# zhm1205/Multimodal_TTA

Hardware: AMD Instinct MI355X
Metric: adapted volumes/sec (higher is better)
Workload: dtype bf16

## Files before the change

include/mmtta.h:

```cpp
#ifndef MMTTA_H
#define MMTTA_H

#include <stdint.h>

#ifdef __cplusplus
extern "C" {
#endif

#define MMTTA_ABI_VERSION 2

typedef enum {
  MMTTA_OK = 0,
  MMTTA_ERR_INVALID = -1,
  MMTTA_ERR_UNSUPPORTED = -2,
  MMTTA_ERR_LAUNCH = -3,
  MMTTA_ERR_WORKSPACE = -4
} mmtta_status;

typedef enum { MMTTA_F32 = 0, MMTTA_BF16 = 1 } mmtta_dtype;

typedef struct {
  void* ptr;
  int32_t n, c, d, h, w;
  int64_t sn, sc, sd, sh, sw;
// ... 18 lines not shown
  float negative_slope;
  int32_t _pad2;
} mmtta_norm_on_load;

const char* mmtta_last_error(void);
int mmtta_abi_version(void);

#define MMTTA_OPT_PROFILE_MAIN_KERNEL_ONLY 1
#define MMTTA_OPT_SPLITK_BELOW 2
#define MMTTA_OPT_SPLITK_TARGET 3
#define MMTTA_OPT_WGRAD_WORKGROUPS 4
#define MMTTA_OPT_WGRAD_THIN_SLABS 5
#define MMTTA_OPT_IGEMM_PIPELINE 6
#define MMTTA_OPT_EPILOGUE_VEC16 9
#define MMTTA_OPT_IGEMM_LEAN 10
#define MMTTA_OPT_WGRAD_VECTOR_STAGING 11
#define MMTTA_OPT_CLASS_FUSED_MIN_WORKGROUPS 12
#define MMTTA_OPT_THIN_MFMA 13
#define MMTTA_OPT_IGEMM_FRAGMENT_REUSE 14
#define MMTTA_OPT_LAME_TILED 15
#define MMTTA_OPT_RAW_STAGING 16
#define MMTTA_OPT_HEAD_LOSS_PAIR 17
#define MMTTA_OPT_THIN_LEAN 18
int mmtta_set_option(int key, int value);

int mmtta_copy_strided(const mmtta_tensor* src, const mmtta_tensor* dst, void* stream);

typedef enum {
  MMTTA_CONV_FWD = 0,
  MMTTA_CONV_DGRAD = 1,
  MMTTA_CONVT_FWD = 2,
  MMTTA_CONVT_DGRAD = 3
} mmtta_conv_op;

typedef struct {
  int32_t op;
  int32_t ksize;
  int32_t stride;
  int32_t cin;
  int32_t cout;
  int32_t dtype;
} mmtta_conv_desc;

int64_t mmtta_conv_packed_bytes(const mmtta_conv_desc* desc);

int mmtta_conv_pack_weights(const mmtta_conv_desc* desc, const float* w_master, void* packed, void* stream);
// ... 18 lines not shown
} mmtta_conv_plan_t;

int mmtta_conv_plan(const mmtta_conv_desc* desc, const mmtta_tensor* x, const mmtta_tensor* y,
                    mmtta_conv_plan_t* plan);

typedef struct {
  const mmtta_tensor* add;
  mmtta_norm_on_load add_norm;
} mmtta_conv_epilogue;

int mmtta_conv_run(const mmtta_conv_desc* desc, const mmtta_tensor* x, const mmtta_norm_on_load* x_norm,
                   const void* packed, const float* bias, const mmtta_conv_epilogue* epi,
                   const mmtta_tensor* y, int accumulate, float* stats, void* workspace,
                   int64_t workspace_bytes, void* stream);

int mmtta_conv_route(const mmtta_conv_desc* desc, const mmtta_tensor* x, const mmtta_norm_on_load* x_norm,
                     const mmtta_conv_epilogue* epi, const mmtta_tensor* y, int accumulate, const float* stats);

int mmtta_conv_stages_raw(const mmtta_conv_desc* desc, const mmtta_tensor* x, const mmtta_norm_on_load* x_norm,
                          const mmtta_conv_epilogue* epi, const mmtta_tensor* y, int accumulate, const float* stats);

int mmtta_conv_thin_lean(const mmtta_conv_desc* desc, const mmtta_tensor* x, const mmtta_norm_on_load* x_norm,
                         const mmtta_conv_epilogue* epi, const mmtta_tensor* y, int accumulate, const float* stats);

typedef struct {
  int32_t items_per_set;
  int32_t inner;
  int64_t packed_outer, packed_inner;
  int64_t weight_outer, weight_inner;
  int64_t bias_outer, bias_inner;
} mmtta_param_sets;

int mmtta_conv_run_sets(const mmtta_conv_desc* desc, const mmtta_tensor* x, const mmtta_norm_on_load* x_norm,
                        const void* packed, const float* bias, const mmtta_conv_epilogue* epi,
                        const mmtta_tensor* y, int accumulate, float* stats, void* workspace,
                        int64_t workspace_bytes, const mmtta_param_sets* sets, void* stream);

int mmtta_conv_head_loss_eligible(const mmtta_conv_desc* desc, const mmtta_tensor* x, const mmtta_norm_on_load* x_norm,
                                  const mmtta_conv_epilogue* epi, const mmtta_tensor* y, const mmtta_tensor* dlogits,
                                  int softmax, int per_item);
int64_t mmtta_conv_head_loss_partials(const mmtta_conv_desc* desc, const mmtta_tensor* x, const mmtta_tensor* y);
int mmtta_conv_head_loss_run_sets(const mmtta_conv_desc* desc, const mmtta_tensor* x, const mmtta_norm_on_load* x_norm,
                                  const void* packed, const float* bias, const mmtta_conv_epilogue* epi,
                                  const mmtta_tensor* y, const mmtta_tensor* dlogits, int softmax, int per_item,
                                  double* partial, float* loss, const mmtta_param_sets* sets, void* stream);

// ... 294 lines not shown
```

multimodal_tta_amd/_lib.py:

```python
from __future__ import annotations

import ctypes as C
import os
from typing import Optional, Sequence

import torch

_HERE = os.path.dirname(os.path.abspath(__file__))
LIB_PATH = os.path.join(_HERE, "csrc", "libmmtta.so")

F32, BF16 = 0, 1
CONV_FWD, CONV_DGRAD, CONVT_FWD, CONVT_DGRAD = 0, 1, 2, 3
NORM_INSTANCE, NORM_BATCH, NORM_GROUP = 0, 1, 2


class MmttaError(RuntimeError):
    pass


class Tensor(C.Structure):
    _fields_ = [
        ("ptr", C.c_void_p),
        ("n", C.c_int32), ("c", C.c_int32), ("d", C.c_int32), ("h", C.c_int32), ("w", C.c_int32),
        ("sn", C.c_int64), ("sc", C.c_int64), ("sd", C.c_int64), ("sh", C.c_int64), ("sw", C.c_int64),
# ... 79 lines not shown


_P = C.POINTER
_SIGNATURES = {
    "mmtta_last_error": (C.c_char_p, []),
    "mmtta_abi_version": (C.c_int, []),
    "mmtta_set_option": (C.c_int, [C.c_int, C.c_int]),
    "mmtta_intensity_scratch_bytes": (C.c_int64, [C.c_int]),
    "mmtta_intensity_normalize": (C.c_int, [_P(Tensor), _P(IntensityRule), _P(Tensor), C.c_void_p, C.c_void_p]),
    "mmtta_copy_strided": (C.c_int, [_P(Tensor), _P(Tensor), C.c_void_p]),
    "mmtta_conv_packed_bytes": (C.c_int64, [_P(ConvDesc)]),
    "mmtta_conv_pack_weights": (C.c_int, [_P(ConvDesc), C.c_void_p, C.c_void_p, C.c_void_p]),
    "mmtta_conv_pack_table_bytes": (C.c_int64, [C.c_int]),
    "mmtta_conv_pack_table_build": (C.c_int, [_P(PackItem), C.c_int, C.c_void_p, _P(C.c_int64)]),
    "mmtta_conv_pack_batched": (C.c_int, [C.c_void_p, C.c_int, C.c_int64, C.c_void_p]),
    "mmtta_conv_plan": (C.c_int, [_P(ConvDesc), _P(Tensor), _P(Tensor), _P(ConvPlan)]),
    "mmtta_conv_run": (C.c_int, [_P(ConvDesc), _P(Tensor), _P(NormOnLoad), C.c_void_p, C.c_void_p, _P(ConvEpilogue),
                                 _P(Tensor), C.c_int, C.c_void_p, C.c_void_p, C.c_int64, C.c_void_p]),
    "mmtta_conv_run_sets": (C.c_int, [_P(ConvDesc), _P(Tensor), _P(NormOnLoad), C.c_void_p, C.c_void_p, _P(ConvEpilogue),
                                      _P(Tensor), C.c_int, C.c_void_p, C.c_void_p, C.c_int64, _P(ParamSets), C.c_void_p]),
    "mmtta_conv_route": (C.c_int, [_P(ConvDesc), _P(Tensor), _P(NormOnLoad), _P(ConvEpilogue), _P(Tensor), C.c_int, C.c_void_p]),
    "mmtta_conv_stages_raw": (C.c_int, [_P(ConvDesc), _P(Tensor), _P(NormOnLoad), _P(ConvEpilogue), _P(Tensor), C.c_int, C.c_void_p]),
    "mmtta_conv_thin_lean": (C.c_int, [_P(ConvDesc), _P(Tensor), _P(NormOnLoad), _P(ConvEpilogue), _P(Tensor), C.c_int, C.c_void_p]),
    "mmtta_conv_head_loss_eligible": (C.c_int, [_P(ConvDesc), _P(Tensor), _P(NormOnLoad), _P(ConvEpilogue), _P(Tensor), _P(Tensor),
                                                C.c_int, C.c_int]),
    "mmtta_conv_head_loss_partials": (C.c_int64, [_P(ConvDesc), _P(Tensor), _P(Tensor)]),
    "mmtta_conv_head_loss_run_sets": (C.c_int, [_P(ConvDesc), _P(Tensor), _P(NormOnLoad), C.c_void_p, C.c_void_p, _P(ConvEpilogue),
                                                _P(Tensor), _P(Tensor), C.c_int, C.c_int, C.c_void_p, C.c_void_p, _P(ParamSets),
                                                C.c_void_p]),
    "mmtta_conv_wgrad_workspace_bytes": (C.c_int64, [_P(ConvDesc), _P(Tensor), _P(Tensor)]),
    "mmtta_conv_wgrad_workspace_bytes_sets": (C.c_int64, [_P(ConvDesc), _P(Tensor), _P(Tensor), _P(ParamSets)]),
    "mmtta_conv_wgrad_plan_sets": (C.c_int, [_P(ConvDesc), _P(Tensor), _P(Tensor), _P(ParamSets), _P(C.c_int32)]),
    "mmtta_conv_wgrad_sets": (C.c_int, [_P(ConvDesc), _P(Tensor), _P(NormOnLoad), _P(Tensor), C.c_void_p, C.c_void_p,
                                        C.c_int, C.c_void_p, C.c_int64, _P(ParamSets), C.c_void_p]),
    "mmtta_conv_wgrad_kernel": (C.c_int, [_P(ConvDesc), _P(Tensor), _P(Tensor)]),
    "mmtta_conv_wgrad_stages_raw": (C.c_int, [_P(ConvDesc), _P(Tensor), _P(NormOnLoad), _P(Tensor)]),
    "mmtta_conv_wgrad": (C.c_int, [_P(ConvDesc), _P(Tensor), _P(NormOnLoad), _P(Tensor), C.c_void_p, C.c_void_p,
                                   C.c_int, C.c_void_p, C.c_int64, C.c_void_p]),
    "mmtta_norm_stats_finalize": (C.c_int, [C.c_int, C.c_int, C.c_void_p, C.c_int, C.c_int, C.c_int, C.c_int64,
                                            C.c_float, C.c_int, C.c_void_p, C.c_void_p, C.c_float, C.c_void_p,
                                            C.c_void_p, C.c_void_p, C.c_void_p, C.c_void_p, C.c_void_p, C.c_void_p,
                                            C.c_void_p]),
    "mmtta_norm_stats_finalize_sets": (C.c_int, [C.c_int, C.c_int, C.c_void_p, C.c_int, C.c_int, C.c_int, C.c_int64,
                                                 C.c_float, C.c_int, C.c_void_p, C.c_void_p, C.c_float, C.c_void_p,
                                                 C.c_void_p, C.c_void_p, C.c_void_p, C.c_void_p, C.c_void_p, C.c_void_p,
                                                 C.c_void_p, C.c_void_p, _P(NormSets), C.c_void_p]),
# ... 129 lines not shown
        fn = getattr(lib, name)
        fn.restype = res
        fn.argtypes = args
    if lib.mmtta_abi_version() != 2:
        raise MmttaError("libmmtta.so ABI version mismatch")
    if os.environ.get("MMTTA_NO_PIPE", "0") == "1":
        lib.mmtta_set_option(6, 0)
    if os.environ.get("MMTTA_NO_EPIVEC", "0") == "1":
        lib.mmtta_set_option(9, 0)
    if "MMTTA_WGVEC" in os.environ:
        lib.mmtta_set_option(11, int(os.environ["MMTTA_WGVEC"]))
    if "MMTTA_THINMFMA" in os.environ:
        lib.mmtta_set_option(13, int(os.environ["MMTTA_THINMFMA"]))
    if "MMTTA_CLSFUSE" in os.environ:
        lib.mmtta_set_option(12, int(os.environ["MMTTA_CLSFUSE"]))
    if "MMTTA_LEAN" in os.environ:
        lib.mmtta_set_option(10, int(os.environ["MMTTA_LEAN"]))
    if "MMTTA_RAWSTAGE" in os.environ:
        lib.mmtta_set_option(16, int(os.environ["MMTTA_RAWSTAGE"]))
    if "MMTTA_HEADLOSS" in os.environ:
        lib.mmtta_set_option(17, int(os.environ["MMTTA_HEADLOSS"]))
    if "MMTTA_THINLEAN" in os.environ:
        lib.mmtta_set_option(18, int(os.environ["MMTTA_THINLEAN"]))
    _lib = lib
    return lib


def exported_names() -> Sequence[str]:
    return list(_SIGNATURES)


def check(status: int, what: str = "") -> None:
    if status != 0:
        msg = load().mmtta_last_error().decode("utf-8", "replace")
        raise MmttaError(f"{what or 'libmmtta'} failed with status {status}: {msg}")


def stream_ptr() -> int:
    return int(torch.cuda.current_stream().cuda_stream)


def ptr(t: Optional[torch.Tensor]) -> Optional[int]:
    return None if t is None else int(t.data_ptr())


TENSOR_OWNS_PAD = 1
# ... 30 lines not shown
```

multimodal_tta_amd/csrc/api.hip:

```cpp
#include "common.h"
#include <string.h>

namespace mmtta {
static thread_local char g_err[512] = "";
void set_error(const char* fmt, ...) {
  va_list ap;
  va_start(ap, fmt);
  vsnprintf(g_err, sizeof(g_err), fmt, ap);
  va_end(ap);
}
int g_profile_main_only = 0;
int g_igemm_pipeline = 1;
int g_epilogue_vec = 1;
int g_igemm_lean = 1;
int g_igemm_reuse = 1;
int g_cls_fused_min = 128;
int g_thin_mfma = 2;
int g_wgrad_vec = 1;
int g_lame_tiled = 1;
int g_raw_staging = 3;
int g_head_loss_pair = 3;
int g_thin_lean = 3;
int g_tune[4] = {96, 128, 128, 256};
}

extern "C" int mmtta_set_option(int key, int value) {
  if (key == MMTTA_OPT_PROFILE_MAIN_KERNEL_ONLY) {
    const int prev = mmtta::g_profile_main_only;
    mmtta::g_profile_main_only = value;
    return prev;
  }
  if (key == MMTTA_OPT_WGRAD_VECTOR_STAGING) {
    const int prev = mmtta::g_wgrad_vec;
    mmtta::g_wgrad_vec = value ? 1 : 0;
    return prev;
  }
  if (key == MMTTA_OPT_THIN_MFMA) {
    const int prev = mmtta::g_thin_mfma;
    mmtta::g_thin_mfma = value < 0 ? 0 : (value > 3 ? 3 : value);
    return prev;
  }
  if (key == MMTTA_OPT_CLASS_FUSED_MIN_WORKGROUPS) {
    const int prev = mmtta::g_cls_fused_min;
    mmtta::g_cls_fused_min = value < 0 ? 0 : value;
    return prev;
// ... 13 lines not shown
    mmtta::g_epilogue_vec = value ? 1 : 0;
    return prev;
  }
  if (key == MMTTA_OPT_LAME_TILED) {
    const int prev = mmtta::g_lame_tiled;
    mmtta::g_lame_tiled = value ? 1 : 0;
    return prev;
  }
  if (key == MMTTA_OPT_RAW_STAGING) {
    const int prev = mmtta::g_raw_staging;
    mmtta::g_raw_staging = value & 3;
    return prev;
  }
  if (key == MMTTA_OPT_HEAD_LOSS_PAIR) {
    const int prev = mmtta::g_head_loss_pair;
    mmtta::g_head_loss_pair = value & 3;
    return prev;
  }
  if (key == MMTTA_OPT_THIN_LEAN) {
    const int prev = mmtta::g_thin_lean;
    mmtta::g_thin_lean = value & 3;
    return prev;
  }
  if (key == MMTTA_OPT_IGEMM_PIPELINE) {
    const int prev = mmtta::g_igemm_pipeline;
    mmtta::g_igemm_pipeline = value ? 1 : 0;
    return prev;
  }
  if (key >= MMTTA_OPT_SPLITK_BELOW && key <= MMTTA_OPT_WGRAD_THIN_SLABS) {
    if (value < 1) return MMTTA_ERR_INVALID;
    const int prev = mmtta::g_tune[key - MMTTA_OPT_SPLITK_BELOW];
    mmtta::g_tune[key - MMTTA_OPT_SPLITK_BELOW] = value;
    return prev;
  }
  return MMTTA_ERR_INVALID;
}

extern "C" const char* mmtta_last_error(void) { return mmtta::g_err; }
extern "C" int mmtta_abi_version(void) { return MMTTA_ABI_VERSION; }
```

multimodal_tta_amd/csrc/common.h:

```cpp
#pragma once
#include <hip/hip_runtime.h>
#include <type_traits>
#include <stdint.h>
#include <stdio.h>
#include <stdarg.h>
#include "../../include/mmtta.h"

namespace mmtta {

constexpr int WAVE = 64;

void set_error(const char* fmt, ...);

#define MMTTA_CHECK(cond, code, ...)      \
  do {                                    \
    if (!(cond)) {                        \
      ::mmtta::set_error(__VA_ARGS__);    \
      return (code);                      \
    }                                     \
  } while (0)

inline int launch_status(const char* what) {
  hipError_t e = hipGetLastError();
  if (e != hipSuccess) {
    set_error("%s: %s", what, hipGetErrorString(e));
    return MMTTA_ERR_LAUNCH;
  }
  return MMTTA_OK;
}

extern int g_profile_main_only;
extern int g_igemm_pipeline;
extern int g_wgrad_vec;
extern int g_igemm_lean;
extern int g_igemm_reuse;
extern int g_cls_fused_min;
extern int g_lame_tiled;
extern int g_thin_mfma;
extern int g_epilogue_vec;
extern int g_raw_staging;
extern int g_head_loss_pair;
extern int g_thin_lean;
extern int g_tune[4];

inline bool nl_leaky(const mmtta_norm_on_load* t) { return t != nullptr && t->relu == MMTTA_ACT_LEAKY_RELU; }
inline int nl_act_check(const mmtta_norm_on_load* t, const char* what) {
  MMTTA_CHECK(t == nullptr || (t->relu >= MMTTA_ACT_NONE && t->relu <= MMTTA_ACT_LEAKY_RELU), MMTTA_ERR_INVALID,
              "%s: activation code %d (MMTTA_ACT_NONE, _RELU or _LEAKY_RELU)", what, t ? t->relu : 0);
  MMTTA_CHECK(t == nullptr || t->relu != MMTTA_ACT_LEAKY_RELU || __builtin_isfinite(t->negative_slope), MMTTA_ERR_INVALID,
              "%s: LeakyReLU negative_slope must be finite", what);
  return MMTTA_OK;
}

struct PackImageGeo {
  int A, B, T, Kp, Np, kn_is_ba, plain_bf16;
};
int pack_image_geometry(const mmtta_conv_desc* d, PackImageGeo& g);

#define MMTTA_ACT_BODIES                                                                                                    \
  int conv_run_body(const mmtta_conv_desc* d, const mmtta_tensor* x, const mmtta_norm_on_load* x_norm, const void* packed,  \
                    const float* bias, const mmtta_conv_epilogue* epi, const mmtta_tensor* y, int accumulate, float* stats, \
                    void* workspace, int64_t workspace_bytes, const mmtta_param_sets* sets, void* stream);                \
  int conv_wgrad_body(const mmtta_conv_desc* d, const mmtta_tensor* x, const mmtta_norm_on_load* x_norm,                    \
                      const mmtta_tensor* dy, float* dw, float* db, int accumulate, void* workspace,                        \
                      int64_t workspace_bytes, const mmtta_param_sets* sets, void* stream,                                  \
// ... 437 lines not shown
int channel_partial_rows(const mmtta_tensor* t);
int launch_channel_sums(const mmtta_tensor* x, float* part, hipStream_t s);

bool direct_applicable(const mmtta_conv_desc* d);
long long upconv8_image_bytes(const mmtta_conv_desc* d);
long long chan_frag_bytes(const mmtta_conv_desc* d);
int direct_blocks_per_n(const mmtta_conv_desc* d, const mmtta_tensor* x, const mmtta_tensor* y);
bool pointwise_small_applicable(const mmtta_conv_desc* d, const mmtta_tensor* x, const mmtta_tensor* y, const float* stats,
                                const mmtta_tensor* add, const mmtta_norm_on_load* x_norm);
int pointwise_small_run(const mmtta_tensor* x, const void* packed, int Kp, int Np, const float* bias, const mmtta_tensor* y,
                        int accumulate, const PSets& sets, hipStream_t stream);
bool chan_applicable(const mmtta_conv_desc* d, const mmtta_tensor* x, const mmtta_tensor* y);
int chan_tiles_per_n(const mmtta_tensor* y);
bool chan_lean_applicable(const mmtta_conv_desc* d, const mmtta_tensor* x, const mmtta_norm_on_load* x_norm,
                          const mmtta_conv_epilogue* epi, const mmtta_tensor* y, int accumulate);
int chan_conv_run(const mmtta_conv_desc* d, const mmtta_tensor* x, const mmtta_norm_on_load* x_norm, const void* packed, int Kp,
                  int Np, const float* bias, const mmtta_conv_epilogue* epi, const mmtta_tensor* y, int accumulate, float* stats,
                  const PSets& sets, hipStream_t stream);
int direct_conv_run(const mmtta_conv_desc* d, const mmtta_tensor* x, const mmtta_norm_on_load* x_norm, const void* packed,
                    const float* bias, const mmtta_conv_epilogue* epi, const mmtta_tensor* y, int accumulate, float* stats,
                    const PSets& sets, hipStream_t stream);
bool direct_upconv8_lean(const mmtta_conv_desc* d, const mmtta_tensor* x, const mmtta_norm_on_load* x_norm,
                         const mmtta_conv_epilogue* epi, const mmtta_tensor* y);
bool direct_head_loss_eligible(const mmtta_conv_desc* d, const mmtta_tensor* x, const mmtta_norm_on_load* x_norm,
                               const mmtta_conv_epilogue* epi, const mmtta_tensor* y, const mmtta_tensor* dz, int softmax,
                               int per_item);
int direct_head_loss_run(const mmtta_conv_desc* d, const mmtta_tensor* x, const mmtta_norm_on_load* x_norm, const void* packed,
                         const float* bias, const mmtta_conv_epilogue* epi, const mmtta_tensor* y, const mmtta_tensor* dz,
                         double* partial, float* loss, const PSets& sets, hipStream_t stream);

MMTTA_ACT_NS_CLOSE
}
```

multimodal_tta_amd/csrc/conv3_mfma4_body.h:

```cpp
  constexpr int TY = 8, TX = 64, BZ = TZ + 2, BY = TY + 2, BX = 68, RUNS = BX / 4, NRUN = BZ * BY * RUNS;
  __shared__ uint2 box[BZ * BY * BX];
  __shared__ uint2 wtab[27 * 4];
  __shared__ float red[32];
  const int n = blockIdx.y;
  a.w = pset_packed(a.ps, a.w, n); a.bias = pset_bias(a.ps, a.bias, n);
  const int tid = threadIdx.x, lane = tid & 63;
  const int wave = __builtin_amdgcn_readfirstlane(tid >> 6);
  const int txn = (a.out.w + TX - 1) / TX, tyn = (a.out.h + TY - 1) / TY;
  int t = blockIdx.x;
  const int txi = t % txn; t /= txn;
  const int tyi = t % tyn;
  const int tzi = t / tyn;
  const int oz0 = tzi * TZ, oy0 = tyi * TY, ox0 = txi * TX;
  if (tid < 27 * 4) {
    const int tp = tid >> 2, j = tid & 3;
    const float* wt = a.w + (a.transposed ? 26 - tp : tp) * a.K * 4;
    float wk[4];
#pragma unroll
    for (int k = 0; k < 4; ++k) wk[k] = (k < a.K && j < a.N) ? wt[k * 4 + j] : 0.f;
    wtab[tid] = make_uint2(f32x2_to_bf16x2(wk[0], wk[1]), f32x2_to_bf16x2(wk[2], wk[3]));
  }
  {
    constexpr int NIT = (NRUN + 255) / 256, RND = NIT;
    float sc[4] = {1.f, 1.f, 1.f, 1.f}, sh[4] = {0.f, 0.f, 0.f, 0.f};
    if (HAS_T) nl_coeff_vec<4>(a.tin, n, a.K, 0, sc, sh);
#pragma unroll
    for (int k = 0; k < 4; ++k)
      if (k >= a.K) { sc[k] = 0.f; sh[k] = 0.f; }
    const float relu_lo = act_lo(HAS_T ? a.tin.relu : MMTTA_ACT_ID);
    const float* inb = GBF ? reinterpret_cast<const float*>(reinterpret_cast<const unsigned short*>(a.in.p) + (long long)n * a.in.sn)
                           : a.in.p + (long long)n * a.in.sn;
    const unsigned isw = (unsigned)a.in.sw;
#pragma unroll 1
    for (int j0 = 0; j0 < NIT; j0 += RND) {
      float4 raw[RND][4];
      unsigned okm = 0u;
#pragma unroll
      for (int j = 0; j < RND; ++j) {
        const int v = min(tid + 256 * (j0 + j), NRUN - 1);
        const int bz = v / (BY * RUNS), rem = v - bz * (BY * RUNS), by = rem / RUNS, run = rem - by * RUNS;
        const int iz = oz0 - 1 + bz, iy = oy0 - 1 + by, ix = ox0 - 1 + 4 * run;
        const bool rok = (unsigned)iz < (unsigned)a.in.d && (unsigned)iy < (unsigned)a.in.h;
        const long long rowo = (long long)min(max(iz, 0), a.in.d - 1) * a.in.sd + (long long)min(max(iy, 0), a.in.h - 1) * a.in.sh;
#pragma unroll
// ... 14 lines not shown
#pragma unroll
        for (int q = 0; q < 4; ++q) {
          if constexpr (GBF) {
            const unsigned ux = __float_as_uint(raw[j][q].x), uy = __float_as_uint(raw[j][q].y);
            raw[j][q] = make_float4(bf16_bits_to_f32(ux & 0xffffu), __uint_as_float(ux & 0xffff0000u),
                                    bf16_bits_to_f32(uy & 0xffffu), __uint_as_float(uy & 0xffff0000u));
          }
          const float xs[4] = {raw[j][q].x, raw[j][q].y, raw[j][q].z, raw[j][q].w};
          float v4[4];
#pragma unroll
          for (int k = 0; k < 4; ++k) v4[k] = act_max(fmaf(xs[k], sc[k], sh[k]), relu_lo);
          const unsigned m = ((okm >> (4 * j + q)) & 1u) ? 0xffffffffu : 0u;
          pk[q].x = f32x2_to_bf16x2(v4[0], v4[1]) & m; pk[q].y = f32x2_to_bf16x2(v4[2], v4[3]) & m;
        }
        if (tid + 256 * (j0 + j) < NRUN) {
          const int v = tid + 256 * (j0 + j), brow = v / RUNS, run = v - brow * RUNS;
          uint2* drow = box + brow * BX;
#pragma unroll
          for (int q = 0; q < 4; ++q) drow[run < 16 ? 16 * (run & 3) + 4 * q + (run >> 2) : 64 + q] = pk[q];
        }
      }
    }
  }
  const int jc = lane & 3, blk = lane >> 2;
  float bias = 0.f, asc = 1.f, ash = 0.f;
  if (jc < a.N) {
    if (a.bias) bias = a.bias[jc];
    if (a.add) nl_coeff(a.tadd, n, a.N, jc, asc, ash);
  }
  __syncthreads();
  cs4 wb[27];
#pragma unroll
  for (int tp = 0; tp < 27; ++tp) wb[tp] = __builtin_bit_cast(cs4, wtab[tp * 4 + jc]);
  float ssum = 0.f, ssq = 0.f;
  const int arow = lane & 3;
  const int jl = min(jc, a.N - 1);
  unsigned xoff_o[4], xoff_a[4];
  unsigned xok = 0u;
#pragma unroll
  for (int r = 0; r < 4; ++r) {
    const int ox = ox0 + 16 * r + blk;
    xok |= (ox < a.out.w ? 1u : 0u) << r;
    xoff_o[r] = (unsigned)min(ox, a.out.w - 1) * (unsigned)a.out.sw;
    xoff_a[r] = (unsigned)min(ox, a.out.w - 1) * (unsigned)a.asw;
  }
#ifdef MMTTA_HEAD_LOSS_BODY
  double lacc = 0.0;
  float* const dzn = hl.dbf ? reinterpret_cast<float*>(reinterpret_cast<unsigned short*>(hl.dz) + (long long)n * hl.dsn)
                            : hl.dz + (long long)n * hl.dsn;
#endif
  float addn[2][4], oldn[2][4];
  auto fetch = [&](int rp) {
    const int r0 = rp * 8 + wave * 2;
#pragma unroll
    for (int q = 0; q < 2; ++q) {
      const int oz = min(oz0 + (r0 + q) / TY, a.out.d - 1), oy = min(oy0 + (r0 + q) % TY, a.out.h - 1);
#pragma unroll
      for (int r = 0; r < 4; ++r) { addn[q][r] = 0.f; oldn[q][r] = 0.f; }
      if (a.add) {
        const long long ao = (long long)n * a.asn + (long long)oz * a.asd + (long long)oy * a.ash;
#pragma unroll
        for (int r = 0; r < 4; ++r) addn[q][r] = ld1_t<GBF>(a.add, ao + xoff_a[r] + jl);
      }
      if (a.accumulate) {
        const long long oo = (long long)n * a.out.sn + (long long)oz * a.out.sd + (long long)oy * a.out.sh;
#pragma unroll
        for (int r = 0; r < 4; ++r) oldn[q][r] = ld1_t<GBF>(a.out.p, oo + xoff_o[r] + jl);
      }
    }
  };
  fetch(0);
#pragma unroll 1
  for (int rp = 0; rp < TZ * TY / 8; ++rp) {
    const int r0 = rp * 8 + wave * 2;
    float addc[2][4], oldc[2][4];
#pragma unroll
    for (int q = 0; q < 2; ++q)
#pragma unroll
      for (int r = 0; r < 4; ++r) { addc[q][r] = addn[q][r]; oldc[q][r] = oldn[q][r]; }
    if (rp + 1 < TZ * TY / 8) fetch(rp + 1);
    cf4v acc[2];
    const uint2* ab[2][3];
#pragma unroll
    for (int q = 0; q < 2; ++q) {
      const int zl = (r0 + q) / TY, yl = (r0 + q) % TY;
#pragma unroll
      for (int dx = 0; dx < 3; ++dx) {
        const int xi = 16 * arow + blk + dx;
        ab[q][dx] = box + (zl * BY + yl) * BX + (xi < 64 ? ((xi & 15) << 2) | (xi >> 4) : xi);
      }
      acc[q] = cf4v{0.f, 0.f, 0.f, 0.f};
    }
#pragma unroll
    for (int tp = 0; tp < 27; ++tp) {
      const int toff = ((tp / 9) * BY + (tp / 3) % 3) * BX;
#pragma unroll
      for (int q = 0; q < 2; ++q) {
        const uint2 av = ab[q][tp % 3][toff];
        acc[q] = __builtin_amdgcn_mfma_f32_4x4x4bf16_1k(__builtin_bit_cast(cs4, av), wb[tp], acc[q], 0, 0, 0);
      }
    }
#pragma unroll
    for (int q = 0; q < 2; ++q) {
      const int oz = oz0 + (r0 + q) / TY, oy = oy0 + (r0 + q) % TY;
      const bool rowok = oz < a.out.d && oy < a.out.h;
      const long long orowo = (long long)n * a.out.sn + (long long)min(oz, a.out.d - 1) * a.out.sd + (long long)min(oy, a.out.h - 1) * a.out.sh;
      float* orow = a.out.p + orowo;
#pragma unroll
      for (int r = 0; r < 4; ++r) {
        float v = acc[q][r] + bias;
        if (a.add) v += nl_apply(addc[q][r], asc, ash, a.tadd.relu);
        if (a.accumulate) v += oldc[q][r];
#ifdef MMTTA_HEAD_LOSS_BODY
        {
          float hc, gc;
          bernoulli_entropy_terms(v, hc, gc);
          const int hb = __builtin_bit_cast(int, hc);
          const float h0 = __builtin_bit_cast(float, __builtin_amdgcn_update_dpp(0, hb, 0x00, 0xf, 0xf, true));
          const float h1 = __builtin_bit_cast(float, __builtin_amdgcn_update_dpp(0, hb, 0x55, 0xf, 0xf, true));
          const float h2 = __builtin_bit_cast(float, __builtin_amdgcn_update_dpp(0, hb, 0xaa, 0xf, 0xf, true));
          const float h3 = __builtin_bit_cast(float, __builtin_amdgcn_update_dpp(0, hb, 0xff, 0xf, 0xf, true));
          float h = 0.f;
          h += h0;
          if (a.N > 1) h += h1;
          if (a.N > 2) h += h2;
          if (a.N > 3) h += h3;
          const float gs = jc < a.N ? gc * hl.inv_count : 0.f;
          const float other = __builtin_bit_cast(float, __builtin_amdgcn_update_dpp(0, __builtin_bit_cast(int, gs), 0xb1, 0xf, 0xf, true));
          if (rowok && ((xok >> r) & 1u)) {
            const unsigned go = (((unsigned)oz * (unsigned)a.out.h + (unsigned)oy) * (unsigned)a.out.w + (unsigned)(ox0 + 16 * r + blk)) * 4u + jc;
// ... 6 lines not shown
          }
          continue;
        }
#endif
        if constexpr (GBF) {
          v = jc < a.N ? v : 0.f;
          const float other = __shfl_xor(v, 1, 64);
          if (rowok && ((xok >> r) & 1u)) {
            if (!(jc & 1))
              *reinterpret_cast<unsigned int*>(reinterpret_cast<unsigned short*>(a.out.p) + orowo + xoff_o[r] + jc) = f32x2_to_bf16x2(v, other);
            if (jc < a.N) { ssum += v; ssq += v * v; }
          }
          continue;
        }
        if (rowok && ((xok >> r) & 1u)) {
          if (jc < a.N) {
            orow[xoff_o[r] + jc] = v;
            ssum += v; ssq += v * v;
          } else if (a.out_vec4) {
            orow[xoff_o[r] + jc] = 0.f;
          }
        }
      }
    }
  }
#ifdef MMTTA_HEAD_LOSS_BODY
  {
    lacc = wave_sum_d(lacc);
    if (lane == 0) {
      const unsigned long long bits = __builtin_bit_cast(unsigned long long, lacc);
      red[2 * wave] = __uint_as_float((unsigned)bits); red[2 * wave + 1] = __uint_as_float((unsigned)(bits >> 32));
    }
    __syncthreads();
    if (tid == 0) {
      double t = 0.0;
#pragma unroll
      for (int w = 0; w < 4; ++w)
        t += __builtin_bit_cast(double, (unsigned long long)__float_as_uint(red[2 * w]) | ((unsigned long long)__float_as_uint(red[2 * w + 1]) << 32));
      hl.partial[(long long)n * gridDim.x + blockIdx.x] = t;
    }
    return;
  }
#endif
  if (a.stats != nullptr) {
#pragma unroll
    for (int o = 4; o < 64; o <<= 1) { ssum += __shfl_xor(ssum, o, 64); ssq += __shfl_xor(ssq, o, 64); }
// ... 11 lines not shown
```

multimodal_tta_amd/csrc/conv_direct.hip:

```cpp
#include "common.h"
#ifndef MMTTA_ACT_LEAKY_TU
#include "voxel_loss.h"
#endif

namespace mmtta {
MMTTA_ACT_NS_OPEN

typedef float float2_t __attribute__((ext_vector_type(2)));
typedef __bf16 bf16x2_t __attribute__((ext_vector_type(2)));
typedef __bf16 ubf16x8 __attribute__((ext_vector_type(8)));
typedef float ufloat16 __attribute__((ext_vector_type(16)));

struct DArgs {
  TV in; NL tin;
  TV out;
  const float* w;
  const float* bias;
  const float* add; long long asn, asd, ash, asw; NL tadd;
  int K, N, ksize, stride, transposed, accumulate;
  float* stats; int blocks_per_n;
  PSets ps;
  int out_vec4;
};

// ... 405 lines not shown
  direct_stats<NO>(a, n, ssum, ssq, red);
}

typedef short cs4 __attribute__((ext_vector_type(4)));
typedef float cf4v __attribute__((ext_vector_type(4)));

template <bool HAS_T, int TZ, bool GBF = false>
__global__ __launch_bounds__(256) void conv3_mfma4_kernel(DArgs a) {
#include "conv3_mfma4_body.h"
}

#ifndef MMTTA_ACT_LEAKY_TU
struct HeadLoss {
  float* dz; long long dsn; int dbf;
  float inv_count;
  double* partial;
};
template <bool HAS_T, int TZ>
__global__ __launch_bounds__(256) void conv3_mfma4_loss_kernel(DArgs a, HeadLoss hl) {
  constexpr bool GBF = false;
#define MMTTA_HEAD_LOSS_BODY
#include "conv3_mfma4_body.h"
#undef MMTTA_HEAD_LOSS_BODY
}
#endif

template <int K, int NO, bool HAS_T>
__global__ __launch_bounds__(256) void direct_upconv_kernel(DArgs a) {
  extern __shared__ float lds[];
  constexpr int VS = K + 4;
  constexpr int XV = 65;
  float* red = lds + 4 * XV * VS;
  const int n = blockIdx.y;
  a.w = pset_packed(a.ps, a.w, n); a.bias = pset_bias(a.ps, a.bias, n);
  cfloat* wc = (cfloat*)a.w;
  const int tid = threadIdx.x, lane = tid & 63;
  const int wave = __builtin_amdgcn_readfirstlane(tid >> 6);
  const int chunks = (a.in.w + 63) / 64;
  int b = blockIdx.x;
  const int chunk = b % chunks; b /= chunks;
  const int iy0 = b % a.in.h;
  const int iz0 = b / a.in.h;
  const int ix0 = chunk * 64;
  {
    constexpr int CG = K / 4;
    constexpr int NIT = (4 * XV * CG + 255) / 256;
// ... 765 lines not shown

template <int K, bool HAS_T>
static void launch_upconv_p(const DArgs& a, int n, bool bf, hipStream_t stream) {
  if (bf) launch_upconv_mfma<K, HAS_T>(a, n, stream); else launch_upconv<K, HAS_T>(a, n, stream);
}

template <bool HAS_T>
static void launch_row(const DArgs& a, int n, hipStream_t stream) {
  switch (a.K) {
    case 1: launch_row_n<1, HAS_T>(a, n, stream); break;
    case 2: launch_row_n<2, HAS_T>(a, n, stream); break;
    case 3: launch_row_n<3, HAS_T>(a, n, stream); break;
    default: launch_row_n<4, HAS_T>(a, n, stream); break;
  }
}

bool direct_upconv8_lean(const mmtta_conv_desc* d, const mmtta_tensor* x, const mmtta_norm_on_load* x_norm,
                         const mmtta_conv_epilogue* epi, const mmtta_tensor* y) {
  const bool has_t = x_norm != nullptr && (x_norm->mean != nullptr || x_norm->scale != nullptr);
  return LEAN_KERNELS && (g_thin_lean & 2) && direct_applicable(d) && direct_variant(d, x) == 5 && is_bf16(x) && !has_t &&
         !nl_leaky(x_norm) && !(epi && epi->add && nl_leaky(&epi->add_norm));
}

int direct_conv_run(const mmtta_conv_desc* d, const mmtta_tensor* x, const mmtta_norm_on_load* x_norm, const void* packed,
                    const float* bias, const mmtta_conv_epilogue* epi, const mmtta_tensor* y, int accumulate, float* stats,
                    const PSets& sets, hipStream_t stream) {
  DArgs a;
  a.ps = sets;
  a.in = tv(x); a.tin = nl(x_norm); a.out = tv(y);
  a.w = (const float*)packed; a.bias = bias;
  const int st = epilogue_add(epi, y, a);
  if (st) return st;
  a.K = x->c; a.N = y->c; a.ksize = d->ksize; a.stride = d->stride;
  a.transposed = (d->op == MMTTA_CONVT_FWD || d->op == MMTTA_CONV_DGRAD) ? 1 : 0;
  a.accumulate = accumulate;
  a.out_vec4 = (y->flags & MMTTA_TENSOR_OWNS_PAD) && y->sw == 4 && aligned16(y);
  a.stats = stats; a.blocks_per_n = direct_blocks_per_n(d, x, y);
  const int T = d->ksize * d->ksize * d->ksize;
  const size_t lds = (size_t)T * a.K * 16 + (size_t)a.K * 8 + 32 * sizeof(float);
  static bool attr_set = false;
  if (!attr_set && lds > 48 * 1024) {
    hipError_t e = hipFuncSetAttribute((const void*)direct_conv_kernel<true>, hipFuncAttributeMaxDynamicSharedMemorySize, 128 * 1024);
    if (e == hipSuccess)
      e = hipFuncSetAttribute((const void*)direct_conv_kernel<false>, hipFuncAttributeMaxDynamicSharedMemorySize, 128 * 1024);
    MMTTA_CHECK(e == hipSuccess, MMTTA_ERR_LAUNCH, "direct conv: cannot raise the dynamic LDS limit: %s", hipGetErrorString(e));
    attr_set = true;
  }
  const bool has_t = a.tin.mean != nullptr || a.tin.scale != nullptr;
  const int variant = direct_variant(d, x);
  const bool thin_bf = variant == 4 && is_bf16(x) && is_bf16(y) && (!(epi && epi->add) || is_bf16(epi->add)) &&
                       x->sw == 4 && y->sw == 4 && ((y->flags & MMTTA_TENSOR_OWNS_PAD) || y->c == 4) && ((uintptr_t)y->ptr) % 8 == 0 &&
                       (!(epi && epi->add) || epi->add->sw == 4);
  MMTTA_CHECK(thin_bf || (is_f32(y) && !(epi && epi->add && is_bf16(epi->add))), MMTTA_ERR_UNSUPPORTED, "direct conv: outputs are fp32-stored");
  if (variant == 5) {
    const int tz = (x->d + 3) / 4, ty = (x->h + 3) / 4, tx = (x->w + 7) / 8;
#ifndef MMTTA_ACT_LEAKY_TU
    if (direct_upconv8_lean(d, x, x_norm, epi, y)) {
      if (a.K == 64) launch_upconv8<64, false, true, true>(a, y->n, tz, ty, tx, stream);
      else launch_upconv8<32, false, true, true>(a, y->n, tz, ty, tx, stream);
      return launch_status("up-convolution (2x2x2 gather GEMM, lean)");
    }
#endif
    MMTTA_BF_DISPATCH(has_t, HT, { MMTTA_BF_DISPATCH(is_bf16(x), XBF, {
      if (a.K == 64) launch_upconv8<64, HT, XBF>(a, y->n, tz, ty, tx, stream);
      else launch_upconv8<32, HT, XBF>(a, y->n, tz, ty, tx, stream);
    }); });
    return launch_status("up-convolution (2x2x2 gather GEMM)");
  }
  MMTTA_CHECK(is_f32(x) || (variant == 3 && d->dtype == MMTTA_BF16) || variant == 1 || thin_bf, MMTTA_ERR_UNSUPPORTED,
              "direct conv: a bf16-stored input is supported by the matrix-core up-convolution and the lanes-along-K kernel only");
  {
    const bool head = d->op == MMTTA_CONV_FWD && d->ksize == 1 && (a.K == 32 || a.K == 64) && !has_t && stats == nullptr &&
                      !(epi && epi->add) && !accumulate && is_f32(y) && dense_rows16(x) && voxel_dense(y) && y->sw == 4 && a.out_vec4;
    if (head) {
      const long long dhw = (long long)y->d * y->h * y->w;
// ... 1 lines not shown
      if (blocks > 2048) blocks = 2048;
      const dim3 grid((unsigned)blocks, y->n), block(256);
      MMTTA_BF_DISPATCH(is_bf16(x), XBF, {
        if (a.K == 32) hipLaunchKernelGGL((pointwise_head_kernel<32, XBF>), grid, block, 0, stream, a);
        else hipLaunchKernelGGL((pointwise_head_kernel<64, XBF>), grid, block, 0, stream, a);
      });
      return launch_status("1x1 head (streaming)");
    }
  }
  if (variant == 1) {
    const size_t kl_lds = (size_t)T * a.K * 16 + 32 * sizeof(float);
    MMTTA_BF_DISPATCH(has_t, HT, {
      if (a.K == 64) launch_klane<16, HT>(a, y->n, kl_lds, stream);
      else launch_klane<8, HT>(a, y->n, kl_lds, stream);
    });
    return launch_status("direct conv (lanes along K)");
  }
  if (variant == 2) {
    MMTTA_BF_DISPATCH(has_t, HT, { launch_row<HT>(a, y->n, stream); });
    return launch_status("direct conv (row)");
  }
  if (variant == 4) {
    const dim3 grid(a.blocks_per_n, y->n), block(256);
    MMTTA_BF_DISPATCH(has_t, HT, { MMTTA_BF_DISPATCH(thin_bf, GBF, {
      switch (g_thin_mfma) {
        case 3: hipLaunchKernelGGL((conv3_mfma4_kernel<HT, 2, GBF>), grid, block, 0, stream, a); break;
        case 2: hipLaunchKernelGGL((conv3_mfma4_kernel<HT, 4, GBF>), grid, block, 0, stream, a); break;
        default: hipLaunchKernelGGL((conv3_mfma4_kernel<HT, 8, GBF>), grid, block, 0, stream, a); break;
      }
    }); });
    return launch_status(thin_bf ? "direct conv (4x4x4 matrix tiles, bf16-stored thin tensors)" : "direct conv (4x4x4 matrix tiles)");
  }
  if (variant == 3) {
    const bool bf = d->dtype == MMTTA_BF16;
    MMTTA_BF_DISPATCH(has_t, HT, {
      if (a.K == 64) launch_upconv_p<64, HT>(a, y->n, bf, stream);
      else launch_upconv_p<32, HT>(a, y->n, bf, stream);
    });
    return launch_status("direct up-convolution");
  }
  MMTTA_BF_DISPATCH(has_t, HT, { hipLaunchKernelGGL(direct_conv_kernel<HT>, dim3(a.blocks_per_n, y->n), dim3(256), lds, stream, a); });
  return launch_status("direct conv");
}

#ifndef MMTTA_ACT_LEAKY_TU
bool direct_head_loss_eligible(const mmtta_conv_desc* d, const mmtta_tensor* x, const mmtta_norm_on_load* x_norm,
// ... 48 lines not shown
```

multimodal_tta_amd/csrc/conv_igemm.hip:

```cpp
#include "common.h"

namespace mmtta {
MMTTA_ACT_NS_OPEN

typedef float f32x16 __attribute__((ext_vector_type(16)));
typedef __bf16 bf16x8 __attribute__((ext_vector_type(8)));
typedef __bf16 bf16x2 __attribute__((ext_vector_type(2)));

__device__ __forceinline__ unsigned int pack_bf16x2(float lo, float hi) {
  bf16x2 v;
  v[0] = (__bf16)lo;
  v[1] = (__bf16)hi;
  return __builtin_bit_cast(unsigned int, v);
}

struct Taps {
  int n;
  int slab[27];
  signed char dz[27], dy[27], dx[27];
  int zmin, ymin, xmin;
  int zext, yext, xext;
};

struct ClassInfo {
// ... 1307 lines not shown
  if (st) return st < 0 ? st : -st;
  return g.route;
}

extern "C" int mmtta_conv_stages_raw(const mmtta_conv_desc* d, const mmtta_tensor* x, const mmtta_norm_on_load* x_norm,
                                     const mmtta_conv_epilogue* epi, const mmtta_tensor* y, int accumulate, const float* stats) {
  Geometry g;
  const int st = plan_run(d, x, x_norm, epi, y, accumulate, stats, nullptr, g);
  if (st) return st < 0 ? st : -st;
  const mmtta_tensor* add = (epi && epi->add) ? epi->add : nullptr;
  return (raw_staging(g.route, g.cfg.bf, x, x_norm, y, add) && !(add && nl_leaky(&epi->add_norm))) ? 1 : 0;
}

extern "C" int mmtta_conv_thin_lean(const mmtta_conv_desc* d, const mmtta_tensor* x, const mmtta_norm_on_load* x_norm,
                                    const mmtta_conv_epilogue* epi, const mmtta_tensor* y, int accumulate, const float* stats) {
  Geometry g;
  const int st = plan_run(d, x, x_norm, epi, y, accumulate, stats, nullptr, g);
  if (st) return st < 0 ? st : -st;
  if (g.route == C_THIN) return chan_lean_applicable(d, x, x_norm, epi, y, accumulate) ? 1 : 0;
  if (g.route == C_DIRECT) return direct_upconv8_lean(d, x, x_norm, epi, y) ? 2 : 0;
  return 0;
}

static int head_loss_plan(const mmtta_conv_desc* d, const mmtta_tensor* x, const mmtta_norm_on_load* x_norm,
                          const mmtta_conv_epilogue* epi, const mmtta_tensor* y, const mmtta_tensor* dz, int softmax, int per_item,
                          bool& eligible) {
  Geometry g;
  const int st = plan_run(d, x, x_norm, epi, y, 0, nullptr, nullptr, g);
  if (st) return st;
  eligible = g.route == C_DIRECT && direct_head_loss_eligible(d, x, x_norm, epi, y, dz, softmax, per_item);
  return MMTTA_OK;
}

extern "C" int mmtta_conv_head_loss_eligible(const mmtta_conv_desc* d, const mmtta_tensor* x, const mmtta_norm_on_load* x_norm,
                                             const mmtta_conv_epilogue* epi, const mmtta_tensor* y, const mmtta_tensor* dlogits,
                                             int softmax, int per_item) {
  bool ok = false;
  const int st = head_loss_plan(d, x, x_norm, epi, y, dlogits, softmax, per_item, ok);
  if (st) return st < 0 ? st : -st;
  return ok ? 1 : 0;
}

extern "C" int64_t mmtta_conv_head_loss_partials(const mmtta_conv_desc* d, const mmtta_tensor* x, const mmtta_tensor* y) {
  Geometry g;
  if (geometry(d, x, y, nullptr, g) || g.route != C_DIRECT) return -1;
  return (int64_t)direct_blocks_per_n(d, x, y) * y->n;
// ... 54 lines not shown
```

Baseline: 115.6.

## Add lean specialized thin 4-channel direct conv kernel for bf16 backward path

Adds a specialized variant of the 4x4x4 MFMA thin direct-conv kernel for bf16 tensors with no input normalization, accumulation or stats. Input staging loads raw 16-byte vectors with bitmask boundary handling instead of per-element normalize-and-convert. When the residual add aliases the input, the add values are taken from the centre tap already held in registers through DPP lane shuffles instead of being reloaded from global memory. The output is packed to bf16 across lanes with DPP and written as one 8-byte store. It is on by default behind an option flag, and the eligibility checks add some code complexity and risk of layout mismatches.

```diff
diff --git a/include/mmtta.h b/include/mmtta.h
--- a/include/mmtta.h
+++ b/include/mmtta.h
@@ -64,6 +64,7 @@
 #define MMTTA_OPT_RAW_STAGING 16
 #define MMTTA_OPT_HEAD_LOSS_PAIR 17
 #define MMTTA_OPT_THIN_LEAN 18
+#define MMTTA_OPT_THIN_BWD_LEAN 19
 int mmtta_set_option(int key, int value);
 
 int mmtta_copy_strided(const mmtta_tensor* src, const mmtta_tensor* dst, void* stream);
@@ -128,6 +129,9 @@
 
 int mmtta_conv_thin_lean(const mmtta_conv_desc* desc, const mmtta_tensor* x, const mmtta_norm_on_load* x_norm,
                          const mmtta_conv_epilogue* epi, const mmtta_tensor* y, int accumulate, const float* stats);
+
+int mmtta_conv_thin_bwd_lean(const mmtta_conv_desc* desc, const mmtta_tensor* x, const mmtta_norm_on_load* x_norm,
+                             const mmtta_conv_epilogue* epi, const mmtta_tensor* y, int accumulate, const float* stats);
 
 typedef struct {
   int32_t items_per_set;
diff --git a/multimodal_tta_amd/_lib.py b/multimodal_tta_amd/_lib.py
--- a/multimodal_tta_amd/_lib.py
+++ b/multimodal_tta_amd/_lib.py
@@ -125,6 +125,7 @@
     "mmtta_conv_route": (C.c_int, [_P(ConvDesc), _P(Tensor), _P(NormOnLoad), _P(ConvEpilogue), _P(Tensor), C.c_int, C.c_void_p]),
     "mmtta_conv_stages_raw": (C.c_int, [_P(ConvDesc), _P(Tensor), _P(NormOnLoad), _P(ConvEpilogue), _P(Tensor), C.c_int, C.c_void_p]),
     "mmtta_conv_thin_lean": (C.c_int, [_P(ConvDesc), _P(Tensor), _P(NormOnLoad), _P(ConvEpilogue), _P(Tensor), C.c_int, C.c_void_p]),
+    "mmtta_conv_thin_bwd_lean": (C.c_int, [_P(ConvDesc), _P(Tensor), _P(NormOnLoad), _P(ConvEpilogue), _P(Tensor), C.c_int, C.c_void_p]),
     "mmtta_conv_head_loss_eligible": (C.c_int, [_P(ConvDesc), _P(Tensor), _P(NormOnLoad), _P(ConvEpilogue), _P(Tensor), _P(Tensor),
                                                 C.c_int, C.c_int]),
     "mmtta_conv_head_loss_partials": (C.c_int64, [_P(ConvDesc), _P(Tensor), _P(Tensor)]),
@@ -300,6 +301,8 @@
         lib.mmtta_set_option(17, int(os.environ["MMTTA_HEADLOSS"]))
     if "MMTTA_THINLEAN" in os.environ:
         lib.mmtta_set_option(18, int(os.environ["MMTTA_THINLEAN"]))
+    if "MMTTA_THINBWD" in os.environ:
+        lib.mmtta_set_option(19, int(os.environ["MMTTA_THINBWD"]))
     _lib = lib
     return lib
 
diff --git a/multimodal_tta_amd/csrc/api.hip b/multimodal_tta_amd/csrc/api.hip
--- a/multimodal_tta_amd/csrc/api.hip
+++ b/multimodal_tta_amd/csrc/api.hip
@@ -21,6 +21,7 @@
 int g_raw_staging = 3;
 int g_head_loss_pair = 3;
 int g_thin_lean = 3;
+int g_thin_bwd_lean = 15;
 int g_tune[4] = {96, 128, 128, 256};
 }
 
@@ -80,6 +81,11 @@
     mmtta::g_thin_lean = value & 3;
     return prev;
   }
+  if (key == MMTTA_OPT_THIN_BWD_LEAN) {
+    const int prev = mmtta::g_thin_bwd_lean;
+    mmtta::g_thin_bwd_lean = value & 15;
+    return prev;
+  }
   if (key == MMTTA_OPT_IGEMM_PIPELINE) {
     const int prev = mmtta::g_igemm_pipeline;
     mmtta::g_igemm_pipeline = value ? 1 : 0;
diff --git a/multimodal_tta_amd/csrc/common.h b/multimodal_tta_amd/csrc/common.h
--- a/multimodal_tta_amd/csrc/common.h
+++ b/multimodal_tta_amd/csrc/common.h
@@ -41,6 +41,7 @@
 extern int g_raw_staging;
 extern int g_head_loss_pair;
 extern int g_thin_lean;
+extern int g_thin_bwd_lean;
 extern int g_tune[4];
 
 inline bool nl_leaky(const mmtta_norm_on_load* t) { return t != nullptr && t->relu == MMTTA_ACT_LEAKY_RELU; }
@@ -524,6 +525,8 @@
                     const PSets& sets, hipStream_t stream);
 bool direct_upconv8_lean(const mmtta_conv_desc* d, const mmtta_tensor* x, const mmtta_norm_on_load* x_norm,
                          const mmtta_conv_epilogue* epi, const mmtta_tensor* y);
+int direct_thin_bwd_lean(const mmtta_conv_desc* d, const mmtta_tensor* x, const mmtta_norm_on_load* x_norm,
+                         const mmtta_conv_epilogue* epi, const mmtta_tensor* y, int accumulate, const float* stats);
 bool direct_head_loss_eligible(const mmtta_conv_desc* d, const mmtta_tensor* x, const mmtta_norm_on_load* x_norm,
                                const mmtta_conv_epilogue* epi, const mmtta_tensor* y, const mmtta_tensor* dz, int softmax,
                                int per_item);
diff --git a/multimodal_tta_amd/csrc/conv3_mfma4_body.h b/multimodal_tta_amd/csrc/conv3_mfma4_body.h
--- a/multimodal_tta_amd/csrc/conv3_mfma4_body.h
+++ b/multimodal_tta_amd/csrc/conv3_mfma4_body.h
@@ -20,6 +20,53 @@
     for (int k = 0; k < 4; ++k) wk[k] = (k < a.K && j < a.N) ? wt[k * 4 + j] : 0.f;
     wtab[tid] = make_uint2(f32x2_to_bf16x2(wk[0], wk[1]), f32x2_to_bf16x2(wk[2], wk[3]));
   }
+#ifdef MMTTA_CONV3_LEAN_BODY
+  {
+    typedef unsigned int u4 __attribute__((ext_vector_type(4)));
+    typedef u4 u4a8 __attribute__((aligned(8)));
+    constexpr int NIT = (NRUN + 255) / 256;
+    const unsigned short* inb = reinterpret_cast<const unsigned short*>(a.in.p) + (long long)n * a.in.sn;
+    const unsigned km0 = a.K > 1 ? 0xffffffffu : 0x0000ffffu;
+    const unsigned km1 = a.K > 3 ? 0xffffffffu : (a.K > 2 ? 0x0000ffffu : 0u);
+    u4 raw[NIT][2];
+    unsigned okm = 0u, upm = 0u, dnm = 0u;
+#pragma unroll
+    for (int j = 0; j < NIT; ++j) {
+      const int v = min(tid + 256 * j, NRUN - 1);
+      const int bz = v / (BY * RUNS), rem = v - bz * (BY * RUNS), by = rem / RUNS, run = rem - by * RUNS;
+      const int iz = oz0 - 1 + bz, iy = oy0 - 1 + by, ix = ox0 - 1 + 4 * run;
+      const bool rok = (unsigned)iz < (unsigned)a.in.d && (unsigned)iy < (unsigned)a.in.h;
+      const long long rowo = (long long)min(max(iz, 0), a.in.d - 1) * a.in.sd + (long long)min(max(iy, 0), a.in.h - 1) * a.in.sh;
+#pragma unroll
+      for (int p = 0; p < 2; ++p) {
+        const int xs = ix + 2 * p, cs = min(max(xs, 0), a.in.w - 2);
+        okm |= ((rok && (unsigned)xs < (unsigned)a.in.w) ? 1u : 0u) << (4 * j + 2 * p);
+        okm |= ((rok && (unsigned)(xs + 1) < (unsigned)a.in.w) ? 1u : 0u) << (4 * j + 2 * p + 1);
+        upm |= (cs > xs ? 1u : 0u) << (2 * j + p);
+        dnm |= (cs < xs ? 1u : 0u) << (2 * j + p);
+        raw[j][p] = *reinterpret_cast<const u4a8*>(inb + rowo + (long long)cs * 4);
+      }
+    }
+#pragma unroll
+    for (int j = 0; j < NIT; ++j) {
+      uint2 pk[4];
+#pragma unroll
+      for (int p = 0; p < 2; ++p) {
+        const bool up = (upm >> (2 * j + p)) & 1u, dn = (dnm >> (2 * j + p)) & 1u;
+        const unsigned m0 = ((okm >> (4 * j + 2 * p)) & 1u) ? 0xffffffffu : 0u, m1 = ((okm >> (4 * j + 2 * p + 1)) & 1u) ? 0xffffffffu : 0u;
+        const u4 u = raw[j][p];
+        pk[2 * p].x = (dn ? u.z : u.x) & m0 & km0; pk[2 * p].y = (dn ? u.w : u.y) & m0 & km1;
+        pk[2 * p + 1].x = (up ? u.x : u.z) & m1 & km0; pk[2 * p + 1].y = (up ? u.y : u.w) & m1 & km1;
+      }
+      if (tid + 256 * j < NRUN) {
+        const int v = tid + 256 * j, brow = v / RUNS, run = v - brow * RUNS;
+        uint2* drow = box + brow * BX;
+#pragma unroll
+        for (int q = 0; q < 4; ++q) drow[run < 16 ? 16 * (run & 3) + 4 * q + (run >> 2) : 64 + q] = pk[q];
+      }
+    }
+  }
+#else
   {
     constexpr int NIT = (NRUN + 255) / 256, RND = NIT;
     float sc[4] = {1.f, 1.f, 1.f, 1.f}, sh[4] = {0.f, 0.f, 0.f, 0.f};
@@ -80,6 +127,7 @@
       }
     }
   }
+#endif
   const int jc = lane & 3, blk = lane >> 2;
   float bias = 0.f, asc = 1.f, ash = 0.f;
   if (jc < a.N) {
@@ -115,7 +163,11 @@
       const int oz = min(oz0 + (r0 + q) / TY, a.out.d - 1), oy = min(oy0 + (r0 + q) % TY, a.out.h - 1);
 #pragma unroll
       for (int r = 0; r < 4; ++r) { addn[q][r] = 0.f; oldn[q][r] = 0.f; }
+#ifdef MMTTA_CONV3_LEAN_BODY
+      if (a.add && !alias) {
+#else
       if (a.add) {
+#endif
         const long long ao = (long long)n * a.asn + (long long)oz * a.asd + (long long)oy * a.ash;
 #pragma unroll
         for (int r = 0; r < 4; ++r) addn[q][r] = ld1_t<GBF>(a.add, ao + xoff_a[r] + jl);
@@ -149,12 +201,18 @@
       }
       acc[q] = cf4v{0.f, 0.f, 0.f, 0.f};
     }
+#ifdef MMTTA_CONV3_LEAN_BODY
+    uint2 ctr[2];
+#endif
 #pragma unroll
     for (int tp = 0; tp < 27; ++tp) {
       const int toff = ((tp / 9) * BY + (tp / 3) % 3) * BX;
 #pragma unroll
       for (int q = 0; q < 2; ++q) {
         const uint2 av = ab[q][tp % 3][toff];
+#ifdef MMTTA_CONV3_LEAN_BODY
+        if (tp == 13) ctr[q] = av;
+#endif
         acc[q] = __builtin_amdgcn_mfma_f32_4x4x4bf16_1k(__builtin_bit_cast(cs4, av), wb[tp], acc[q], 0, 0, 0);
       }
     }
@@ -164,6 +222,40 @@
       const bool rowok = oz < a.out.d && oy < a.out.h;
       const long long orowo = (long long)n * a.out.sn + (long long)min(oz, a.out.d - 1) * a.out.sd + (long long)min(oy, a.out.h - 1) * a.out.sh;
       float* orow = a.out.p + orowo;
+#ifdef MMTTA_CONV3_LEAN_BODY
+      {
+        float vv[4];
+#define MMTTA_LEAN_ADD(r, ctl)                                                                                             \
+        {                                                                                                                  \
+          float v = acc[q][r] + bias;                                                                                      \
+          if (a.add) {                                                                                                     \
+            float ad = addc[q][r];                                                                                         \
+            if (alias) {                                                                                                   \
+              const unsigned bx = (unsigned)__builtin_amdgcn_update_dpp(0, (int)ctr[q].x, ctl, 0xf, 0xf, true);            \
+              const unsigned by = (unsigned)__builtin_amdgcn_update_dpp(0, (int)ctr[q].y, ctl, 0xf, 0xf, true);            \
+              const unsigned sel = (jl & 2) ? by : bx;                                                                     \
+              ad = __uint_as_float((jl & 1) ? (sel & 0xffff0000u) : (sel << 16));                                          \
+            }                                                                                                              \
+            v += nl_apply(ad, asc, ash, a.tadd.relu);                                                                      \
+          }                                                                                                                \
+          vv[r] = jc < a.N ? v : 0.f;                      \
+        }
+        MMTTA_LEAN_ADD(0, 0x00) MMTTA_LEAN_ADD(1, 0x55) MMTTA_LEAN_ADD(2, 0xaa) MMTTA_LEAN_ADD(3, 0xff)
+#undef MMTTA_LEAN_ADD
+        const unsigned p01 = f32x2_to_bf16x2(vv[0], vv[1]), p23 = f32x2_to_bf16x2(vv[2], vv[3]);
+        const bool hi2 = (jc & 2) != 0, odd = (jc & 1) != 0;
+        const unsigned got = (unsigned)__builtin_amdgcn_update_dpp(0, (int)(hi2 ? p01 : p23), 0x4e, 0xf, 0xf, true);
+        const unsigned ca = hi2 ? got : p01;
+        const unsigned cb = hi2 ? p23 : got;
+        const unsigned pa = (unsigned)__builtin_amdgcn_update_dpp(0, (int)ca, 0xb1, 0xf, 0xf, true);
+        const unsigned pb = (unsigned)__builtin_amdgcn_update_dpp(0, (int)cb, 0xb1, 0xf, 0xf, true);
+        uint2 o;
+        o.x = odd ? ((pa >> 16) | (ca & 0xffff0000u)) : ((ca & 0xffffu) | (pa << 16));
+        o.y = odd ? ((pb >> 16) | (cb & 0xffff0000u)) : ((cb & 0xffffu) | (pb << 16));
+        if (rowok && ox0 + 16 * jc + blk < a.out.w)
+          *reinterpret_cast<uint2*>(reinterpret_cast<unsigned short*>(a.out.p) + orowo + (unsigned)(ox0 + 16 * jc + blk) * 4u) = o;
+      }
+#else
 #pragma unroll
       for (int r = 0; r < 4; ++r) {
         float v = acc[q][r] + bias;
@@ -216,6 +308,7 @@
           }
         }
       }
+#endif
     }
   }
 #ifdef MMTTA_HEAD_LOSS_BODY
diff --git a/multimodal_tta_amd/csrc/conv_direct.hip b/multimodal_tta_amd/csrc/conv_direct.hip
--- a/multimodal_tta_amd/csrc/conv_direct.hip
+++ b/multimodal_tta_amd/csrc/conv_direct.hip
@@ -451,6 +451,15 @@
 #define MMTTA_HEAD_LOSS_BODY
 #include "conv3_mfma4_body.h"
 #undef MMTTA_HEAD_LOSS_BODY
+}
+
+template <int TZ>
+__global__ __launch_bounds__(256) void conv3_mfma4_lean_kernel(DArgs a, int alias) {
+  constexpr bool HAS_T = false, GBF = true;
+  a.accumulate = 0; a.stats = nullptr;
+#define MMTTA_CONV3_LEAN_BODY
+#include "conv3_mfma4_body.h"
+#undef MMTTA_CONV3_LEAN_BODY
 }
 #endif
 
@@ -1262,6 +1271,25 @@
          !nl_leaky(x_norm) && !(epi && epi->add && nl_leaky(&epi->add_norm));
 }
 
+static bool thin_bf_tensors(const mmtta_tensor* x, const mmtta_tensor* y, const mmtta_tensor* add) {
+  return is_bf16(x) && is_bf16(y) && (!add || is_bf16(add)) && x->sw == 4 && y->sw == 4 &&
+         ((y->flags & MMTTA_TENSOR_OWNS_PAD) || y->c == 4) && ((uintptr_t)y->ptr) % 8 == 0 && (!add || add->sw == 4);
+}
+
+int direct_thin_bwd_lean(const mmtta_conv_desc* d, const mmtta_tensor* x, const mmtta_norm_on_load* x_norm,
+                         const mmtta_conv_epilogue* epi, const mmtta_tensor* y, int accumulate, const float* stats) {
+  const mmtta_tensor* add = (epi && epi->add) ? epi->add : nullptr;
+  const bool has_t = x_norm != nullptr && (x_norm->mean != nullptr || x_norm->scale != nullptr);
+  if (!LEAN_KERNELS || !(g_thin_bwd_lean & 1) || !direct_applicable(d) || direct_variant(d, x) != 4) return 0;
+  if (!thin_bf_tensors(x, y, add) || has_t || accumulate || stats != nullptr) return 0;
+  if (nl_leaky(x_norm) || (add && nl_leaky(&epi->add_norm))) return 0;
+  if (x->w < 2 || x->sc != 1 || y->sc != 1 || y->sn % 4 || y->sd % 4 || y->sh % 4) return 0;
+  const bool alias = add && add->ptr == x->ptr && add->sn == x->sn && add->sd == x->sd && add->sh == x->sh &&
+                     add->sw == x->sw && add->sc == x->sc && add->dtype == x->dtype && x->c == y->c &&
+                     epi->add_norm.mean == nullptr && epi->add_norm.scale == nullptr && epi->add_norm.relu == MMTTA_ACT_NONE;
+  return alias ? 2 : 1;
+}
+
 int direct_conv_run(const mmtta_conv_desc* d, const mmtta_tensor* x, const mmtta_norm_on_load* x_norm, const void* packed,
                     const float* bias, const mmtta_conv_epilogue* epi, const mmtta_tensor* y, int accumulate, float* stats,
                     const PSets& sets, hipStream_t stream) {
@@ -1288,9 +1316,7 @@
   }
   const bool has_t = a.tin.mean != nullptr || a.tin.scale != nullptr;
   const int variant = direct_variant(d, x);
-  const bool thin_bf = variant == 4 && is_bf16(x) && is_bf16(y) && (!(epi && epi->add) || is_bf16(epi->add)) &&
-                       x->sw == 4 && y->sw == 4 && ((y->flags & MMTTA_TENSOR_OWNS_PAD) || y->c == 4) && ((uintptr_t)y->ptr) % 8 == 0 &&
-                       (!(epi && epi->add) || epi->add->sw == 4);
+  const bool thin_bf = variant == 4 && thin_bf_tensors(x, y, (epi && epi->add) ? epi->add : nullptr);
   MMTTA_CHECK(thin_bf || (is_f32(y) && !(epi && epi->add && is_bf16(epi->add))), MMTTA_ERR_UNSUPPORTED, "direct conv: outputs are fp32-stored");
   if (variant == 5) {
     const int tz = (x->d + 3) / 4, ty = (x->h + 3) / 4, tx = (x->w + 7) / 8;
@@ -1338,6 +1364,17 @@
   }
   if (variant == 4) {
     const dim3 grid(a.blocks_per_n, y->n), block(256);
+#ifndef MMTTA_ACT_LEAKY_TU
+    if (const int lean = direct_thin_bwd_lean(d, x, x_norm, epi, y, accumulate, stats)) {
+      const int alias = lean == 2 ? 1 : 0;
+      switch (g_thin_mfma) {
+        case 3: hipLaunchKernelGGL((conv3_mfma4_lean_kernel<2>), grid, block, 0, stream, a, alias); break;
+        case 2: hipLaunchKernelGGL((conv3_mfma4_lean_kernel<4>), grid, block, 0, stream, a, alias); break;
+        default: hipLaunchKernelGGL((conv3_mfma4_lean_kernel<8>), grid, block, 0, stream, a, alias); break;
+      }
+      return launch_status("direct conv (4x4x4 matrix tiles, bf16-stored thin tensors, lean)");
+    }
+#endif
     MMTTA_BF_DISPATCH(has_t, HT, { MMTTA_BF_DISPATCH(thin_bf, GBF, {
       switch (g_thin_mfma) {
         case 3: hipLaunchKernelGGL((conv3_mfma4_kernel<HT, 2, GBF>), grid, block, 0, stream, a); break;
diff --git a/multimodal_tta_amd/csrc/conv_igemm.hip b/multimodal_tta_amd/csrc/conv_igemm.hip
--- a/multimodal_tta_amd/csrc/conv_igemm.hip
+++ b/multimodal_tta_amd/csrc/conv_igemm.hip
@@ -1353,6 +1353,14 @@
   return 0;
 }
 
+extern "C" int mmtta_conv_thin_bwd_lean(const mmtta_conv_desc* d, const mmtta_tensor* x, const mmtta_norm_on_load* x_norm,
+                                        const mmtta_conv_epilogue* epi, const mmtta_tensor* y, int accumulate, const float* stats) {
+  Geometry g;
+  const int st = plan_run(d, x, x_norm, epi, y, accumulate, stats, nullptr, g);
+  if (st) return st < 0 ? st : -st;
+  return g.route == C_DIRECT ? direct_thin_bwd_lean(d, x, x_norm, epi, y, accumulate, stats) : 0;
+}
+
 static int head_loss_plan(const mmtta_conv_desc* d, const mmtta_tensor* x, const mmtta_norm_on_load* x_norm,
                           const mmtta_conv_epilogue* epi, const mmtta_tensor* y, const mmtta_tensor* dz, int softmax, int per_item,
                           bool& eligible) {
```

After: 116.0, median of 4. About the same (+0.3%).
